# lenskit/csr

Measured on AMD Instinct MI355X. Metric: spmv_gflops, higher is better.
Workload: dtype f64

## Files before the change

### csr_amd/csrc/spmv.hip

```cpp
#include "spmv_plan.h"

#include <algorithm>
#include <ctime>

namespace csrk {
template <bool R32>
__device__ __forceinline__ double spmv_prod(double a, double x)
{
    const double t = a * x;
    return R32 ? (double)(float)t : t;
}

void free_spmv_plan(SpmvPlan *p) { delete p; }

void spmv_plan_bytes_by_part(const SpmvPlan *p, int64_t out[5])
{
    for (int i = 0; i < 5; i++) out[i] = 0;
    auto add = [&](int part, std::initializer_list<const DevBuf *> bufs) {
        for (const DevBuf *b : bufs) out[part] += (int64_t)b->bytes;
    };
    for (const AccPanel *ap : p->acc) add(0, {&ap->row_list, &ap->vals, &ap->idx, &ap->tile_row0, &ap->segs, &ap->wg_seg, &ap->partial, &ap->z});
    const Panel &t = p->tier1;
    add(1, {&t.row_list, &t.rp, &t.ci, &t.vs, &t.tile, &t.group, &t.carry_row, &t.carry_val, &t.y, &t.crp, &t.cidx});
    const LightStream *l = &p->ls;
// ... 369 lines not shown
                int q = atomicAdd(&s_nlong, 1);
                s_long[q] = r;
                continue;
            }
            double acc = ordered_sum(s_prod, s, e);
            if (r < nr) {
                yp[i0 + r] = acc;
            } else {
                *(pt.cslot >= 0 ? yp + pt.cslot : carry_val + t) = acc;
            }
        }
        __syncthreads();
        const int nlong = s_nlong;
        for (int q = wv; q < nlong; q += PT / WAVE) {
            int r = s_long[q];
            int s = r ? s_rend[r - 1] : 0;
            int e = s_rend[r];
            double acc = 0.0;
            for (int k = s + lane; k < e; k += WAVE) acc += s_prod[k];
            acc = wave_sum(acc);
            if (lane == 0) {
                if (r < nr) {
                    yp[i0 + r] = acc;
                } else {
                    *(pt.cslot >= 0 ? yp + pt.cslot : carry_val + t) = acc;
                }
            }
        }
        pt = nx;
    }
#undef PANEL_LOAD_TILE
}

typedef float f32x4_t __attribute__((ext_vector_type(4)));
template <class SV> struct AccVals;
template <> struct AccVals<double> {
    f64x2_t v[4];
    __device__ __forceinline__ void load(const double *tile, int lane)
    {
        const f64x2_t *vp = (const f64x2_t *)tile;
#pragma unroll
        for (int q = 0; q < 4; q++) v[q] = __builtin_nontemporal_load(vp + q * WAVE + lane);
    }
    __device__ __forceinline__ void get(double (&a)[ACC_K]) const
    {
#pragma unroll
        for (int q = 0; q < 4; q++) {
            a[2 * q] = v[q].x;
            a[2 * q + 1] = v[q].y;
        }
    }
};
template <> struct AccVals<float> {
    f32x4_t v[2];
    __device__ __forceinline__ void load(const float *tile, int lane)
    {
        const f32x4_t *vp = (const f32x4_t *)tile;
#pragma unroll
        for (int q = 0; q < 2; q++) v[q] = __builtin_nontemporal_load(vp + q * WAVE + lane);
    }
    __device__ __forceinline__ void get(double (&a)[ACC_K]) const
    {
#pragma unroll
        for (int q = 0; q < 2; q++) {
            a[4 * q] = (double)v[q].x;
            a[4 * q + 1] = (double)v[q].y;
            a[4 * q + 2] = (double)v[q].z;
            a[4 * q + 3] = (double)v[q].w;
        }
    }
};

template <int CB, int PT, bool R32 = false, class SV = double, class XT = double>
__global__ __launch_bounds__(PT) void spmv_acc_kernel(const SV *__restrict__ pvals, const uint16_t *__restrict__ pidx,
                                                     const int32_t *__restrict__ tile_row0,
                                                     const XT *__restrict__ x, int32_t ncols,
                                                     const AccSeg *__restrict__ segs, const int32_t *__restrict__ wg_seg,
                                                     int32_t H, double *__restrict__ partial)
{
    extern __shared__ __align__(16) unsigned char acc_smem[];
    double *s_x = (double *)acc_smem;
    double *s_acc = s_x + CB + 2;
    const int Hpad = (H + 1) & ~1;
    double *s_hval = s_acc + Hpad;
    int32_t *s_hrow = (int32_t *)(s_hval + ACC_SEG_TILES);
    constexpr int NW = PT / WAVE;
    const int tid = threadIdx.x, lane = tid & (WAVE - 1), wv = tid / WAVE;

    for (int h = tid; h < Hpad; h += PT) s_acc[h] = 0.0;
    if (tid < 2) s_x[CB + tid] = 0.0;
    const unsigned long long below = lane ? (~0ull >> (WAVE - lane)) : 0ull;
    const unsigned long long upto = below | (1ull << lane);

    int cur_blk = -1;
    const int sb = wg_seg[blockIdx.x], se = wg_seg[blockIdx.x + 1];
    for (int si = sb; si < se; si++) {
        const AccSeg sg = segs[si];
        if (sg.blk != cur_blk) {
            cur_blk = sg.blk;
            const int32_t w0 = sg.blk * CB;
            const int wlen = ncols - w0 < CB ? ncols - w0 : CB;
            if (wlen == CB) {
                constexpr int WL = CB / 2 / PT;
                f64x2_t v[WL];
#pragma unroll
                for (int u = 0; u < WL; u++) {
                    if (sizeof(XT) == 8) {
                        v[u] = *((const F64x2 *)(x + w0) + tid + u * PT);
                    } else {
                        const f32x2_t t = *((const F32x2 *)(x + w0) + tid + u * PT);
                        v[u].x = (double)t.x;
// ... 1 lines not shown
                    }
                }
#pragma unroll
                for (int u = 0; u < WL; u++) ((f64x2_t *)s_x)[tid + u * PT] = v[u];
            } else {
                for (int k = tid; k < wlen; k += PT) s_x[k] = (double)x[w0 + k];
            }
        }
        __syncthreads();

        const int nt = sg.ntiles;
        AccVals<SV> v, vn;
        u32x4_t ix, ixn;
        int32_t tr0 = 0, tr0n = 0;
        int t = wv;
        const int64_t pstep = (int64_t)gridDim.x;
        if (t < nt) {
            const u32x4_t *ip = (const u32x4_t *)(pidx + (sg.ptile0 + t * pstep) * ACC_TILE);
            v.load(pvals + (sg.ptile0 + t * pstep) * ACC_TILE, lane);
            ix = __builtin_nontemporal_load(ip + lane);
            tr0 = tile_row0[sg.tile0 + t];
        }
        for (; t < nt; t += NW) {
            const bool more = t + NW < nt;
            if (more) {
                const u32x4_t *ip = (const u32x4_t *)(pidx + (sg.ptile0 + (t + NW) * pstep) * ACC_TILE);
                vn.load(pvals + (sg.ptile0 + (t + NW) * pstep) * ACC_TILE, lane);
                ixn = __builtin_nontemporal_load(ip + lane);
                tr0n = tile_row0[sg.tile0 + t + NW];
            }
            const uint32_t e[ACC_K] = {ix.x & 0xffffu, ix.x >> 16, ix.y & 0xffffu, ix.y >> 16,
                                       ix.z & 0xffffu, ix.z >> 16, ix.w & 0xffffu, ix.w >> 16};
            double a[ACC_K];
            v.get(a);
            double xv[ACC_K];
#pragma unroll
            for (int j = 0; j < ACC_K; j++) xv[j] = s_x[e[j] & ACC_COL_MASK];
            int rw[ACC_K];
            {
                int lsum = 0;
#pragma unroll
                for (int j = 0; j < ACC_K; j++) lsum += (int)(e[j] >> ACC_ROW_SHIFT);
                int run = tr0 + wave_exscan_i32(lsum, lane);
#pragma unroll
                for (int j = 0; j < ACC_K; j++) {
                    run += (int)(e[j] >> ACC_ROW_SHIFT);
                    rw[j] = run;
                }
            }
            const int hr = rw[0];
            int cur = hr;
            double acc = 0.0, hs = 0.0;
            bool nb = false;
#pragma unroll
            for (int j = 0; j < ACC_K; j++) {
                const int r = rw[j];
                if (r != cur) {
                    if (!nb) {
                        hs = acc;
                        nb = true;
                    } else {
                        atomicAdd(&s_acc[cur], acc);
                    }
                    acc = 0.0;
                    cur = r;
                }
                if (R32) acc += spmv_prod<true>(a[j], xv[j]);
// ... 511 lines not shown
                dn[q] = k < k1 ? __builtin_nontemporal_load(a_dst + k) : 0;
            }
        }
#pragma unroll
        for (int q = 0; q < LS_STAGE_IPT; q++)
            if (c[q] >= 0) xg[d[q]] = s_x[c[q]];
        if (kn < k1) {
#pragma unroll
            for (int q = 0; q < LS_STAGE_IPT; q++) c[q] = cn[q], d[q] = dn[q];
        }
    }
}

int spmv_kernel_attributes()
{
    for (const void *f : {(const void *)spmv_acc_kernel<ACC_CB, ACC_THREADS>, (const void *)spmv_lstream_kernel<LS_PLAIN>,
                          (const void *)spmv_lstream_kernel<LS_RND>, (const void *)spmv_lstream_kernel<LS_PLAIN, true>,
                          (const void *)spmv_lstream_kernel<LS_RND, true>, (const void *)spmv_acc_kernel<ACC_CB, ACC_THREADS, true>,
                          (const void *)spmv_lstream_kernel<LS_PLAIN, false, true>, (const void *)spmv_lstream_kernel<LS_RND, false, true>,
                          (const void *)spmv_lstream_kernel<LS_PLAIN, true, true>, (const void *)spmv_lstream_kernel<LS_RND, true, true>,
                          (const void *)spmv_acc_kernel<ACC_CB, ACC_THREADS, false, float>,
                          (const void *)spmv_acc_kernel<ACC_CB, ACC_THREADS, true, float>,
                          (const void *)spmv_lstream_kernel<LS_PLAIN, false, false, float>, (const void *)spmv_lstream_kernel<LS_RND, false, false, float>,
                          (const void *)spmv_lstream_kernel<LS_PLAIN, true, false, float>, (const void *)spmv_lstream_kernel<LS_RND, true, false, float>,
                          (const void *)spmv_lstream_kernel<LS_PLAIN, false, true, float>, (const void *)spmv_lstream_kernel<LS_RND, false, true, float>,
                          (const void *)spmv_lstream_kernel<LS_PLAIN, true, true, float>, (const void *)spmv_lstream_kernel<LS_RND, true, true, float>,
                          (const void *)spmv_lstream_kernel<LS_RND24>, (const void *)spmv_lstream_kernel<LS_RND24, true>,
                          (const void *)spmv_lstream_kernel<LS_RND24, false, true>, (const void *)spmv_lstream_kernel<LS_RND24, true, true>,
                          (const void *)spmv_lstream_kernel<LS_RND24, false, false, float>, (const void *)spmv_lstream_kernel<LS_RND24, true, false, float>,
                          (const void *)spmv_lstream_kernel<LS_RND24, false, true, float>, (const void *)spmv_lstream_kernel<LS_RND24, true, true, float>,
                          (const void *)spmv_acc_kernel<ACC_CB, ACC_THREADS, false, double, float>,
                          (const void *)spmv_acc_kernel<ACC_CB, ACC_THREADS, true, double, float>,
                          (const void *)spmv_acc_kernel<ACC_CB, ACC_THREADS, false, float, float>,
                          (const void *)spmv_acc_kernel<ACC_CB, ACC_THREADS, true, float, float>})
        CSRK_HIP(hipFuncSetAttribute(f, hipFuncAttributeMaxDynamicSharedMemorySize, (int)(160 * 1024)));
    CSRK_HIP(hipFuncSetAttribute((const void *)ls_stage_kernel<double>, hipFuncAttributeMaxDynamicSharedMemorySize, (int)(LS_STAGE_WMAX * 8)));
    CSRK_HIP(hipFuncSetAttribute((const void *)ls_stage_kernel<float>, hipFuncAttributeMaxDynamicSharedMemorySize, (int)(LS_STAGE_WMAX * 8)));
    return CSRK_OK;
}

static int get_plan_locked(Matrix *m, hipStream_t s, SpmvPlan **out, bool launching)
{
    if (launching) m->spmv_calls++;
    const char *env = getenv("CSRK_SPMV_HEAVY_SPLIT"), *env_hot = getenv("CSRK_SPMV_HOT"), *env_ls = getenv("CSRK_SPMV_STREAM");
    const bool eager = (env && env[0] == '1') || (env_hot && env_hot[0] == '1') || (env_ls && env_ls[0] == '1') || !launching;
    const bool want_split = eager || m->spmv_calls >= 2;
    if (m->spmv_plan && !m->spmv_plan->split_considered && want_split && m->spmv_plan->algo == CSRK_SPMV_MERGE &&
        !m->spmv_plan->profiling) {
        if (hipDeviceSynchronize() != hipSuccess) {
            set_error("device synchronisation failed: %s", hipGetErrorString(hipGetLastError()));
            return CSRK_ERR_HIP;
        }
        free_spmv_plan(m->spmv_plan);
        m->spmv_plan = nullptr;
    }
    if (!m->spmv_plan) {
        SpmvPlan *p = new (std::nothrow) SpmvPlan();
        CSRK_REQUIRE(p, "out of host memory");
        p->algo = m->spmv_algo == CSRK_SPMV_AUTO ? CSRK_SPMV_MERGE : m->spmv_algo;
        (void)s;
        int rc = build_spmv_plan(m, p, want_split);
        if (rc == CSRK_OK && hipDeviceSynchronize() != hipSuccess) {
            set_error("SpMV plan construction failed: %s", hipGetErrorString(hipGetLastError()));
            rc = CSRK_ERR_HIP;
        }
        if (rc != CSRK_OK) {
            delete p;
// ... 54 lines not shown
            EpiJob J = {};
            J.kind = 1;
            J.blocks = (int32_t)ceil_div(H, WAVE * (EPI_THREADS / WAVE / G));
            J.partial = part;
            J.row_list = rows;
            J.H = H;
            J.n_wg = n_wg;
            J.G = G;
            J.extra = extra;
            J.crp = crp;
            J.cidx = cidx;
            J.cval = cval;
            epi.j[epi.n++] = J;
            return CSRK_OK;
        };
        if (do_light && p->ls.on && p->ls.n_cold) {
            KernelTimer ks(p, s, 3);
            const unsigned gs = (unsigned)(ceil_div(p->ls.n_stage_blk, 8) * 8);
            ls_stage_kernel<XT><<<gs, LS_STAGE_THREADS, (size_t)p->ls.stage_w * 8, s>>>(
                d_x, m->ncols, p->ls.stage_w, p->ls.a_col.as<uint16_t>(), p->ls.a_dst.as<int32_t>(),
                p->ls.blk_start.as<int32_t>(), p->ls.n_stage_blk, p->ls.xg.as<double>());
            ks.stop();
            CSRK_LAUNCH_CHECK();
        }
        if (do_light && p->n_hot && !(p->ls.on && p->ls.n_cold)) {
            hot_pack_kernel<XT><<<(unsigned)ceil_div(p->n_hot, 256), 256, 0, s>>>(d_x, p->hot_cols.as<int32_t>(), p->n_hot,
                                                                            p->xh.as<double>());
            CSRK_LAUNCH_CHECK();
        }
        bool t0_rides = false;
        if (do_heavy && p->n_heavy && !p->acc.empty()) {
            KernelTimer kh(p, s, 1);
            for (AccPanel *ap : p->acc) {
                if (ap->f32)
                    spmv_acc_kernel<ACC_CB, ACC_THREADS, R32, float, XT><<<(unsigned)ap->n_wg, ACC_THREADS, ap->lds, s>>>(
                        ap->vals.as<float>(), ap->idx.as<uint16_t>(), ap->tile_row0.as<int32_t>(), d_x, m->ncols,
                        ap->segs.as<AccSeg>(), ap->wg_seg.as<int32_t>(), ap->nrow, ap->partial.as<double>());
                else
                    spmv_acc_kernel<ACC_CB, ACC_THREADS, R32, double, XT><<<(unsigned)ap->n_wg, ACC_THREADS, ap->lds, s>>>(
                        ap->vals.as<double>(), ap->idx.as<uint16_t>(), ap->tile_row0.as<int32_t>(), d_x, m->ncols,
                        ap->segs.as<AccSeg>(), ap->wg_seg.as<int32_t>(), ap->nrow, ap->partial.as<double>());
                CSRK_LAUNCH_CHECK();
            }
            kh.stop();
        }
        if (do_heavy && p->n_heavy && p->tier1.on) {
            Panel *pn = &p->tier1;
            KernelTimer kh(p, s, 2);
#define PANEL_ARGS(PP)                                                                                              \
    pn->rp.as<PP>(), pn->ci.as<int32_t>(), pn->vs.as<double>(), d_x, m->ncols, pn->y.as<double>(),                    \
        pn->tile.as<PanelTile>(), pn->group.as<PanelGroup>(), pn->rows, pn->carry_row.as<int32_t>(),                  \
        pn->carry_val.as<double>(), pn->nnz, pn->cb, rider
            PanelRider rider = {pn->groups, nullptr, nullptr, 0, 0};
            if (PANEL_T1 / WAVE == 4 && do_heavy && p->acc.size() == 1 && p->acc[0]->z.p) {
                AccPanel *ap = p->acc[0];
                rider.partial = ap->partial.as<double>();
                rider.z = ap->z.as<double>();
                rider.H = ap->nrow;
                rider.n_wg = ap->n_wg;
                t0_rides = true;
            }
            const unsigned grid = (unsigned)(pn->groups + (t0_rides ? ceil_div(rider.H, WAVE) : 0));
            if (pn->p64) spmv_panel_kernel<int64_t, PANEL_T1, R32, XT><<<grid, PANEL_T1, 0, s>>>(PANEL_ARGS(int64_t));
            else spmv_panel_kernel<int32_t, PANEL_T1, R32, XT><<<grid, PANEL_T1, 0, s>>>(PANEL_ARGS(int32_t));
#undef PANEL_ARGS
            kh.stop();
            CSRK_LAUNCH_CHECK();
        }
        if (do_light) {
#define MERGE_ARGS_LIGHT(CI)                                                                                        \
    p->rp_light.as<P>(), CI, m->d_values, d_x, d_y, p->tile_row.as<int32_t>(), m->nrows, p->nnz_light,                \
        p->carry_row.as<int32_t>(), p->carry_val.as<double>(), p->tile_cut.as<int32_t>(), p->cut_pos.as<int64_t>(),  \
        p->cut_cum.as<int64_t>(), m->nnz
#define MERGE_ARGS_FULL(CI)                                                                                         \
// ... 457 lines not shown
```

### csr_amd/csrc/spmv_plan.h

```cpp
#pragma once
#include "common.h"
#include "wave.h"

#include <vector>

namespace csrk {

template <int VT> struct ValLoad;
template <> struct ValLoad<CSRK_VAL_F64> {
    static __device__ __forceinline__ double at(const void *v, int64_t k) { return ((const double *)v)[k]; }
};
template <> struct ValLoad<CSRK_VAL_F32> {
    static __device__ __forceinline__ double at(const void *v, int64_t k) { return (double)((const float *)v)[k]; }
};
template <> struct ValLoad<CSRK_VAL_NONE> {
    static __device__ __forceinline__ double at(const void *, int64_t) { return 1.0; }
};

__device__ __forceinline__ double wave_sum(double v)
{
#pragma unroll
    for (int off = WAVE / 2; off > 0; off >>= 1) v += __shfl_down(v, off, WAVE);
    return v;
}

__device__ __forceinline__ double ordered_sum(const double *p, int s, int e)
{
    double acc = 0.0;
    int k = s;
    for (; k + 4 <= e; k += 4) {
        const double a = p[k], b = p[k + 1], c = p[k + 2], d = p[k + 3];
        acc += a;
        acc += b;
        acc += c;
        acc += d;
    }
    for (; k < e; k++) acc += p[k];
    return acc;
}

struct Panel {
    bool on = false, p64 = false;
    int32_t cb = 0, nb = 0, nrow = 0;
    int64_t rows = 0, tiles = 0, nnz = 0, groups = 0;
    DevBuf row_list;
    DevBuf rp, ci, vs, tile, group, carry_row, carry_val, y;
    int32_t ncs = 0;
    DevBuf crp, cidx;
};

struct AccSeg {
    int64_t tile0;
    int64_t ptile0;
    int32_t ntiles;
    int32_t blk;
};

struct AccPanel {
    int32_t nrow = 0, nb = 0, n_wg = 0;
    int64_t tiles = 0, nnz = 0, n_segs = 0;
    size_t lds = 0;
    DevBuf row_list, vals, idx, tile_row0, segs, wg_seg, partial;
    DevBuf z;
    bool f32 = false;
};

struct LightStream {
    bool on = false;
    int64_t n_tiles = 0;
    int32_t n_runs = 0, n_out = 0;
    unsigned grid = 0;
    DevBuf vals, idx, rowids, tile_base, carry_row, carry_val;
    bool idx24 = false;
    bool f32 = false;
    bool dense = false;
    int64_t n_cold = 0;
    int32_t n_stage_blk = 0, stage_w = 0;
    DevBuf xg, a_col, a_dst, blk_start;
    int32_t stage_tiles = 0;
    DevBuf round_start, round_tile0, wg_round0;
};

struct SpmvPlan {
    int algo = CSRK_SPMV_MERGE;
    int tile_items = 0;
    int64_t n_tiles = 0;
    DevBuf tile_row;
    DevBuf carry_row;
    DevBuf carry_val;
    bool split_considered = false;
    int32_t n_heavy = 0;
    int32_t heavy_min = 0;
    int32_t tier1_min = 0;
    int64_t nnz_light = 0;
    DevBuf rp_light;
    DevBuf cut_pos;
    DevBuf cut_cum;
// ... 93 lines not shown
    int64_t t0;
    int32_t nt;
    int32_t blk;
};
constexpr int ACC_CB = 4096;
constexpr int ACC_K = 8;
constexpr int ACC_TILE = WAVE * ACC_K;
constexpr int ACC_MAXROWS = 15936;
constexpr int ACC_FLOOR = 128;
constexpr int ACC_SEG_TILES = 256;
constexpr int ACC_THREADS = 1024;
constexpr int ACC_ROW_SHIFT = 13;
constexpr uint32_t ACC_COL_MASK = (1u << ACC_ROW_SHIFT) - 1;
constexpr int ACC_MAXSTEP = 7;

typedef uint32_t u32x4_t __attribute__((ext_vector_type(4)));
typedef uint32_t u32x2_t __attribute__((ext_vector_type(2)));

__host__ __device__ __forceinline__ int acc_val_slot(int e)
{
    const int lane = e >> 3, j = e & 7;
    return (j >> 1) * (2 * WAVE) + lane * 2 + (j & 1);
}
__host__ __device__ __forceinline__ int acc_idx_slot(int e)
{
    const int lane = e >> 3, j = e & 7;
    return (j >> 2) * (4 * WAVE) + lane * 4 + (j & 3);
}
template <class SV> __host__ __device__ __forceinline__ int acc_slot_of(int e)
{
    return sizeof(SV) == 8 ? acc_val_slot(e) : acc_idx_slot(e);
}

#ifndef CSRK_LS_THREADS
#define CSRK_LS_THREADS 512
#endif
constexpr int LS_THREADS = CSRK_LS_THREADS;
#ifndef CSRK_LS_HOT_LDS
#define CSRK_LS_HOT_LDS 15360
#endif
constexpr int LS_HOT_LDS = CSRK_LS_HOT_LDS;
#ifndef CSRK_LS_RND_CAP
#define CSRK_LS_RND_CAP 8192
#endif
constexpr int LS_RND_CAP = CSRK_LS_RND_CAP, LS_RND_MAXTILES = 128;
constexpr int LS_RND_HOT = (160 * 1024 - (CSRK_LS_THREADS / 64) * (512 + 2) * 8) / 8 - LS_RND_CAP;
constexpr int LS_RID = 4;
#ifndef CSRK_LS_SEQ
#define CSRK_LS_SEQ 3
#endif
constexpr int LS_SEQ = CSRK_LS_SEQ;
constexpr uint32_t LS_HOT_BIT = 1u << 31, LS_START_BIT = 1u << 30, LS_COL_MASK = (1u << 30) - 1;
constexpr uint32_t LS_PAD = LS_COL_MASK;
#ifndef CSRK_LS_IDX24
#define CSRK_LS_IDX24 1
#endif
constexpr uint32_t LS24_HOT_BIT = 1u << 23, LS24_COL_MASK = (1u << 22) - 1;
constexpr int LS24_START_SHIFT = 22;
constexpr int64_t LS24_TILE_BYTES = 512 * 3;

constexpr int VEC_SEG = 4096;


#ifndef CSRK_STAGE_TILES
#define CSRK_STAGE_TILES 8
#endif
// ... 11 lines not shown
```

### csr_amd/csrc/spmv_plan.hip

```cpp
#include "spmv_plan.h"

#include <algorithm>
#include <cstring>
#include <ctime>

namespace csrk {
struct PlanTrace {
    bool on;
    double t0;
    static double now()
    {
        timespec ts;
        clock_gettime(CLOCK_MONOTONIC, &ts);
        return ts.tv_sec * 1e3 + ts.tv_nsec * 1e-6;
    }
    PlanTrace() : on(getenv("CSRK_PLAN_TRACE") != nullptr), t0(0.0)
    {
        if (on) {
            (void)hipDeviceSynchronize();
            t0 = now();
        }
    }
    void lap(const char *what)
    {
        if (!on) return;
        (void)hipDeviceSynchronize();
        const double t = now();
        fprintf(stderr, "[csrk plan] %-28s %8.3f ms\n", what, t - t0);
        t0 = t;
    }
};

template <class P>
__global__ void merge_plan_kernel(const P *__restrict__ rp, int32_t nrows, int64_t nnz, int items,
                                  int64_t n_tiles, int32_t *__restrict__ tile_row)
{
    int64_t t = (int64_t)blockIdx.x * blockDim.x + threadIdx.x;
// ... 461 lines not shown

__global__ __launch_bounds__(256) void acc_gap_kernel(int64_t *__restrict__ cnt, int32_t n_heavy, int32_t n_blocks,
                                                     int32_t *__restrict__ gap)
{
    const int64_t b = ((int64_t)blockIdx.x * blockDim.x + threadIdx.x) / WAVE;
    const int lane = threadIdx.x & (WAVE - 1);
    if (b >= n_blocks) return;
    int32_t last = -1;
    for (int32_t c0 = 0; c0 < n_heavy; c0 += WAVE) {
        const int32_t c = c0 + lane;
        const bool present = c < n_heavy && cnt[b * n_heavy + c] > 0;
        const unsigned long long mask = __ballot(present);
        const unsigned long long below = lane ? (mask & (~0ull >> (WAVE - lane))) : 0ull;
        const int32_t prev = below ? c0 + 63 - __clzll((long long)below) : last;
        if (c < n_heavy) {
            const int32_t g = present && prev >= 0 ? c - prev : 0;
            gap[b * n_heavy + c] = g;
            if (g > ACC_MAXSTEP) cnt[b * n_heavy + c] += (g - 1) / ACC_MAXSTEP;
        }
        if (mask) last = c0 + 63 - __clzll((long long)mask);
    }
}

__device__ __forceinline__ int64_t acc_phys_tile(int64_t t, const int64_t *__restrict__ wg_t0, int32_t n_wg)
{
    const int64_t n_tiles = wg_t0[n_wg];
    int64_t w = (int64_t)((double)t * (double)n_wg / (double)(n_tiles > 0 ? n_tiles : 1));
    w = w > n_wg - 1 ? n_wg - 1 : (w < 0 ? 0 : w);
    while (w > 0 && wg_t0[w] > t) w--;
    while (w + 1 < n_wg && wg_t0[w + 1] <= t) w++;
    return (t - wg_t0[w]) * n_wg + w;
}

template <class P, int VT, class SV>
__global__ __launch_bounds__(256) void acc_fill_kernel(const P *__restrict__ rp, const int32_t *__restrict__ ci,
                                                      const void *__restrict__ vs, const int32_t *__restrict__ heavy_row,
                                                      int32_t n_heavy, int32_t n_blocks, int32_t cb,
                                                      const int64_t *__restrict__ off, const int64_t *__restrict__ blk_tile0,
                                                      const int32_t *__restrict__ pstart, const int32_t *__restrict__ gap,
                                                      SV *__restrict__ pvals, uint16_t *__restrict__ pidx,
                                                      int32_t *__restrict__ tile_row0, const int64_t *__restrict__ wg_t0,
                                                      int32_t n_wg, int32_t waves_per_block)
{
    __shared__ int32_t s_start[256 / WAVE][WAVE];
    const int64_t w = ((int64_t)blockIdx.x * blockDim.x + threadIdx.x) / WAVE;
    const int lane = threadIdx.x & (WAVE - 1), wv = threadIdx.x / WAVE;
    const int32_t b = (int32_t)(w / waves_per_block);
    if (b >= n_blocks) return;
    const int32_t c0 = (int32_t)(w % waves_per_block) * WAVE, c = c0 + lane;
    const bool valid = c < n_heavy;
    const int64_t i = (int64_t)b * n_heavy + (valid ? c : c0);
    const int64_t off_i = off[i];
    int32_t n_all = 0, g = 0;
    int64_t lo = 0;
    if (valid) {
        n_all = (int32_t)(off[i + 1] - off_i);
        g = gap[i];
        lo = (int64_t)rp[heavy_row[c]] + pstart[i];
    }
    const int32_t npad = g > ACC_MAXSTEP ? (g - 1) / ACC_MAXSTEP : 0;
    const int32_t start = wave_exscan_i32(n_all, lane);
    const int32_t total = __builtin_amdgcn_readlane(start + n_all, WAVE - 1);
    if (total == 0) return;
    const int64_t L0 = blk_tile0[b] * ACC_TILE + (__shfl(off_i, 0, WAVE) - off[(int64_t)b * n_heavy]);
    int32_t *starts = s_start[wv];
    starts[lane] = start;
    __builtin_amdgcn_wave_barrier();
    for (int32_t d0 = 0; d0 < total; d0 += WAVE) {
        const int32_t d = d0 + lane;
        const bool in = d < total;
        int p = 0;
#pragma unroll
        for (int step = WAVE / 2; step; step >>= 1)
            if (in && starts[p + step] <= d) p += step;
        const int32_t at = d - __shfl(start, p, WAVE);
        const int32_t npad_p = __shfl(npad, p, WAVE), g_p = __shfl(g, p, WAVE);
        const int64_t lo_p = __shfl(lo, p, WAVE);
        if (!in) continue;
        const int64_t L = L0 + d;
        const int64_t t = L / ACC_TILE;
        const int el = (int)(L % ACC_TILE);
        const int64_t pt = acc_phys_tile(t, wg_t0, n_wg);
        if (at < npad_p) {
            pvals[pt * ACC_TILE + acc_slot_of<SV>(el)] = (SV)0.0;
            pidx[pt * ACC_TILE + el] = (uint16_t)((uint32_t)cb | ((el ? (uint32_t)ACC_MAXSTEP : 0u) << ACC_ROW_SHIFT));
            if (el == 0) tile_row0[t] = c0 + p - g_p + ACC_MAXSTEP * (at + 1);
        } else {
            const int64_t k = lo_p + (at - npad_p);
            const uint32_t step_in = at == npad_p ? (uint32_t)(g_p - ACC_MAXSTEP * npad_p) : 0u;
            pvals[pt * ACC_TILE + acc_slot_of<SV>(el)] = (SV)ValLoad<VT>::at(vs, k);
            pidx[pt * ACC_TILE + el] = (uint16_t)((uint32_t)(ci[k] - b * cb) | ((el ? step_in : 0u) << ACC_ROW_SHIFT));
            if (el == 0) tile_row0[t] = c0 + p;
        }
    }
}

template <class SV>
__global__ __launch_bounds__(256) void acc_pad_kernel(const int64_t *__restrict__ off, int32_t n_heavy, int32_t n_blocks,
                                                     const int64_t *__restrict__ blk_tile0, SV *__restrict__ pvals,
                                                     uint16_t *__restrict__ pidx, const int64_t *__restrict__ wg_t0, int32_t n_wg)
{
    const int32_t b = blockIdx.x;
    if (b >= n_blocks) return;
    const int64_t cnt = off[(int64_t)(b + 1) * n_heavy] - off[(int64_t)b * n_heavy];
    const int64_t L0 = blk_tile0[b] * ACC_TILE + cnt, L1 = blk_tile0[b + 1] * ACC_TILE;
    for (int64_t L = L0 + threadIdx.x; L < L1; L += blockDim.x) {
        const int64_t pt = acc_phys_tile(L / ACC_TILE, wg_t0, n_wg);
        const int el = (int)(L % ACC_TILE);
        pvals[pt * ACC_TILE + acc_slot_of<SV>(el)] = (SV)0.0;
        pidx[pt * ACC_TILE + el] = (uint16_t)ACC_CB;
    }
}


template <class P>
__device__ __forceinline__ int32_t ls_row_of(const P *__restrict__ rpv, int32_t nrows, int64_t L)
{
    int32_t lo = 0, hi = nrows - 1;
    while (lo < hi) {
        const int32_t mid = lo + ((hi - lo) >> 1);
        if ((int64_t)rpv[mid + 1] > L)
            hi = mid;
        else
            lo = mid + 1;
    }
    return lo;
}

template <class P>
__global__ void ls_tilerow_kernel(const P *__restrict__ rpv, int32_t nrows, int64_t n_ent, int64_t n_tiles, int32_t *__restrict__ tile_row)
{
    const int64_t t = (int64_t)blockIdx.x * blockDim.x + threadIdx.x;
    if (t > n_tiles) return;
    const int64_t e0 = t * ACC_TILE;
    tile_row[t] = t < n_tiles && e0 < n_ent ? ls_row_of(rpv, nrows, e0) : nrows - 1;
}

template <class P>
__global__ void ls_rowflag_kernel(const P *__restrict__ rpv, int32_t nrows, int32_t *__restrict__ flag)
{
    const int64_t r = (int64_t)blockIdx.x * blockDim.x + threadIdx.x;
    if (r <= nrows) flag[r] = (r < nrows && rpv[r + 1] > rpv[r]) ? 1 : 0;
}
// ... 252 lines not shown
    tr.lap("  tier 0: pair starts");
    acc_paircount_kernel<<<(unsigned)ceil_div(pairs, 256), 256, 0, s>>>(pstart.as<int32_t>(), pairs, n, off.as<int64_t>());
    CSRK_LAUNCH_CHECK();
    DevBuf gap;
    CSRK_TRY(gap.alloc((size_t)pairs * 4));
    acc_gap_kernel<<<(unsigned)ceil_div((int64_t)nb * WAVE, 256), 256, 0, s>>>(off.as<int64_t>(), n, nb, gap.as<int32_t>());
    CSRK_LAUNCH_CHECK();
    CSRK_TRY(exclusive_scan_i64(off.as<int64_t>(), off.as<int64_t>(), pairs, s));
    CSRK_TRY(bends.alloc((size_t)(nb + 1) * 8));
    panel_blockends_kernel<<<(unsigned)ceil_div(nb + 1, 256), 256, 0, s>>>(off.as<int64_t>(), n, nb, bends.as<int64_t>());
    CSRK_LAUNCH_CHECK();
    std::vector<int64_t> be((size_t)nb + 1), t0((size_t)nb + 1);
    CSRK_TRY(stage_d2h(be.data(), bends.p, (size_t)(nb + 1) * 8, s));
    CSRK_HIP(hipStreamSynchronize(s));
    t0[0] = 0;
    for (int32_t b = 0; b < nb; b++) t0[b + 1] = t0[b] + ceil_div(be[b + 1] - be[b], ACC_TILE);
    const int64_t n_tiles = t0[nb];
    CSRK_TRY(stage_h2d(bends.p, t0.data(), (size_t)(nb + 1) * 8, s));
    tr.lap("  tier 0: counts, gaps, scan");
    int cus = 0;
    CSRK_HIP(hipDeviceGetAttribute(&cus, hipDeviceAttributeMultiprocessorCount, m->device));
    int64_t n_wg = cus > 0 ? cus : 256;
    if (n_wg > n_tiles) n_wg = n_tiles;
    if (n_wg < 1) n_wg = 1;
    std::vector<int64_t> wg_t0((size_t)n_wg + 1);
    int64_t share_max = 0;
    for (int64_t w = 0; w <= n_wg; w++) wg_t0[(size_t)w] = n_tiles * w / n_wg;
    for (int64_t w = 0; w < n_wg; w++) share_max = std::max(share_max, wg_t0[(size_t)w + 1] - wg_t0[(size_t)w]);
    const int64_t n_phys = share_max * n_wg;
    DevBuf d_wg_t0;
    CSRK_TRY(d_wg_t0.alloc((size_t)(n_wg + 1) * 8));
    CSRK_TRY(stage_h2d(d_wg_t0.p, wg_t0.data(), (size_t)(n_wg + 1) * 8, s));
    ap->f32 = VT == CSRK_VAL_F32;
    CSRK_TRY(ap->vals.alloc((size_t)n_phys * ACC_TILE * (ap->f32 ? 4 : 8)));
    CSRK_TRY(ap->idx.alloc((size_t)n_phys * ACC_TILE * 2));
    CSRK_TRY(ap->tile_row0.alloc((size_t)(n_tiles ? n_tiles : 1) * 4));
    const int32_t fill_waves = (int32_t)ceil_div(n, WAVE);
#define ACC_FILL(SV)                                                                                                   \
    do {                                                                                                               \
        acc_fill_kernel<P, VT, SV><<<(unsigned)ceil_div((int64_t)nb * fill_waves * WAVE, 256), 256, 0, s>>>(           \
            rp, m->d_colinds, m->d_values, ap->row_list.as<int32_t>(), n, nb, ACC_CB, off.as<int64_t>(),               \
            bends.as<int64_t>(), pstart.as<int32_t>(), gap.as<int32_t>(), ap->vals.as<SV>(), ap->idx.as<uint16_t>(),   \
            ap->tile_row0.as<int32_t>(), d_wg_t0.as<int64_t>(), (int32_t)n_wg, fill_waves);                            \
        CSRK_LAUNCH_CHECK();                                                                                           \
        acc_pad_kernel<SV><<<(unsigned)nb, 256, 0, s>>>(off.as<int64_t>(), n, nb, bends.as<int64_t>(), ap->vals.as<SV>(), \
                                                        ap->idx.as<uint16_t>(), d_wg_t0.as<int64_t>(), (int32_t)n_wg); \
        CSRK_LAUNCH_CHECK();                                                                                           \
    } while (0)
    if (ap->f32) ACC_FILL(float);
    else ACC_FILL(double);
#undef ACC_FILL
    tr.lap("  tier 0: fill");
    std::vector<AccSeg> segs;
    std::vector<int32_t> wg_seg((size_t)n_wg + 1);
    int32_t b = 0;
    for (int64_t w = 0; w < n_wg; w++) {
        wg_seg[(size_t)w] = (int32_t)segs.size();
        int64_t t = wg_t0[(size_t)w];
        const int64_t t_end = wg_t0[(size_t)w + 1];
        while (t < t_end) {
            while (t0[b + 1] <= t) b++;
            int64_t e = t_end < t0[b + 1] ? t_end : t0[b + 1];
            if (e - t > ACC_SEG_TILES) e = t + ACC_SEG_TILES;
            AccSeg sg;
            sg.tile0 = t;
            sg.ptile0 = (t - wg_t0[(size_t)w]) * n_wg + w;
            sg.ntiles = (int32_t)(e - t);
            sg.blk = b;
            segs.push_back(sg);
            t = e;
        }
    }
    wg_seg[(size_t)n_wg] = (int32_t)segs.size();
    CSRK_TRY(ap->segs.alloc(segs.size() * sizeof(AccSeg)));
    CSRK_TRY(ap->wg_seg.alloc(wg_seg.size() * 4));
    CSRK_TRY(stage_h2d(ap->segs.p, segs.data(), segs.size() * sizeof(AccSeg), s));
    CSRK_TRY(stage_h2d(ap->wg_seg.p, wg_seg.data(), wg_seg.size() * 4, s));
    CSRK_TRY(ap->partial.alloc((size_t)n_wg * n * 8));
    CSRK_TRY(ap->z.alloc((size_t)n * 8));
    ap->lds = (size_t)(ACC_CB + 2) * 8 + (size_t)((n + 1) & ~1) * 8 + (size_t)ACC_SEG_TILES * 12;
    CSRK_TRY(spmv_kernel_attributes());
    CSRK_HIP(hipStreamSynchronize(s));
    ap->nrow = n;
    ap->nb = nb;
    ap->n_wg = (int32_t)n_wg;
// ... 788 lines not shown
```

Baseline: 775.7.

## Pack heavy-tier f64 values into lossless 56-bit fixed-point tiles

Adds a fix56 encoding for the heavy-row accumulator panel: at plan time a kernel scans the f64 values' exponent range, and if all values fit a shared 52-bit fixed-point grid they are stored as 7-byte split planes (lo/mid/hi) instead of 8-byte doubles. The SpMV kernel decodes them with a perm and magic-number subtraction. The goal is to cut value-stream bandwidth in this memory-bound kernel by 12.5%. A verify pass checks bit-exact roundtrip and falls back to plain doubles on mismatch, at the cost of extra plan time and some decode ALU work.

```diff
diff --git a/csr_amd/csrc/fix56.h b/csr_amd/csrc/fix56.h
--- /dev/null
+++ b/csr_amd/csrc/fix56.h
@@ -0,0 +1,119 @@
+#pragma once
+#include <cstdint>
+#include <cstring>
+
+#if defined(__HIPCC__)
+#define FIX56_HD __host__ __device__ __forceinline__
+#else
+#define FIX56_HD inline
+#endif
+
+namespace csrk {
+namespace fix56 {
+
+constexpr int TILE = 512;
+constexpr int LO_BYTES = TILE * 4, MID_BYTES = TILE * 2, HI_BYTES = TILE;
+constexpr int MID_OFF = LO_BYTES, HI_OFF = LO_BYTES + MID_BYTES;
+constexpr int TILE_BYTES = LO_BYTES + MID_BYTES + HI_BYTES;
+constexpr uint64_t MANT_MASK = (1ull << 52) - 1;
+constexpr uint32_t W_MANT = 0x000fffffu, W_SIGN = 0x00800000u;
+
+struct Packed {
+    unsigned char b[7];
+};
+static_assert(sizeof(Packed) * TILE == TILE_BYTES, "a tile of Packed entries is the three planes");
+
+FIX56_HD uint64_t bits_of(double v)
+{
+    uint64_t b;
+    memcpy(&b, &v, 8);
+    return b;
+}
+FIX56_HD double double_of(uint32_t hi, uint32_t lo)
+{
+    const uint64_t b = ((uint64_t)hi << 32) | lo;
+    double v;
+    memcpy(&v, &b, 8);
+    return v;
+}
+FIX56_HD int ctz64(uint64_t x) { return __builtin_ctzll(x); }
+FIX56_HD int msb64(uint64_t x) { return 63 - __builtin_clzll(x); }
+
+struct Range {
+    int32_t bad = 0, lo = INT32_MAX, hi = INT32_MIN;
+};
+FIX56_HD void split(uint64_t bits, uint64_t &sig, int &unit)
+{
+    const int e = (int)((bits >> 52) & 0x7ff);
+    sig = (bits & MANT_MASK) | (e ? 1ull << 52 : 0ull);
+    unit = (e ? e : 1) - 1075;
+}
+FIX56_HD void fold(Range &r, double v)
+{
+    const uint64_t b = bits_of(v);
+    if (b == 0) return;
+    if (((b >> 52) & 0x7ff) == 0x7ff || b == 1ull << 63) {
+        r.bad = 1;
+        return;
+    }
+    uint64_t sig;
+    int unit;
+    split(b, sig, unit);
+    const int lo = unit + ctz64(sig), hi = unit + msb64(sig);
+    r.lo = lo < r.lo ? lo : r.lo;
+    r.hi = hi > r.hi ? hi : r.hi;
+}
+FIX56_HD void merge(Range &r, const Range &o)
+{
+    r.bad |= o.bad;
+    r.lo = o.lo < r.lo ? o.lo : r.lo;
+    r.hi = o.hi > r.hi ? o.hi : r.hi;
+}
+FIX56_HD bool packable(const Range &r, int32_t &g)
+{
+    g = 0;
+    if (r.bad) return false;
+    if (r.lo > r.hi) return true;
+    g = r.lo;
+    return r.hi - g < 52 && 1075 + g >= 1 && 1075 + g <= 2046;
+}
+
+FIX56_HD uint64_t encode(double v, int32_t g)
+{
+    const uint64_t b = bits_of(v);
+    if ((b << 1) == 0) return 0;
+    uint64_t sig;
+    int unit;
+    split(b, sig, unit);
+    const uint64_t M = unit >= g ? sig << (unit - g) : sig >> (g - unit);
+    return M | (b >> 63) << 55;
+}
+FIX56_HD uint32_t lo_of(uint64_t p) { return (uint32_t)p; }
+FIX56_HD uint16_t mid_of(uint64_t p) { return (uint16_t)(p >> 32); }
+FIX56_HD unsigned char hi_of(uint64_t p) { return (unsigned char)(p >> 48); }
+
+FIX56_HD double decode(uint32_t lo, uint32_t w, uint32_t ebits, double magic)
+{
+    const double d = double_of((w & W_MANT) | ebits, lo) - magic;
+    return double_of((uint32_t)(bits_of(d) >> 32) ^ ((w & W_SIGN) << 8), (uint32_t)bits_of(d));
+}
+FIX56_HD uint32_t ebits_of(int32_t g) { return (uint32_t)(1075 + g) << 20; }
+FIX56_HD double magic_of(int32_t g) { return double_of(ebits_of(g), 0u); }
+
+FIX56_HD int lo_slot(int e) { return ((e & 7) >> 2) * 256 + (e >> 3) * 4 + (e & 3); }
+
+FIX56_HD void put(unsigned char *tile, int e, uint64_t p)
+{
+    ((uint32_t *)tile)[lo_slot(e)] = lo_of(p);
+    ((uint16_t *)(tile + MID_OFF))[e] = mid_of(p);
+    tile[HI_OFF + e] = hi_of(p);
+}
+FIX56_HD double get(const unsigned char *tile, int e, int32_t g)
+{
+    const uint32_t lo = ((const uint32_t *)tile)[lo_slot(e)];
+    const uint32_t w = (uint32_t)((const uint16_t *)(tile + MID_OFF))[e] | (uint32_t)tile[HI_OFF + e] << 16;
+    return decode(lo, w, ebits_of(g), magic_of(g));
+}
+
+}
+}
diff --git a/csr_amd/csrc/spmv.hip b/csr_amd/csrc/spmv.hip
--- a/csr_amd/csrc/spmv.hip
+++ b/csr_amd/csrc/spmv.hip
@@ -425,51 +425,12 @@
 #undef PANEL_LOAD_TILE
 }
 
-typedef float f32x4_t __attribute__((ext_vector_type(4)));
-template <class SV> struct AccVals;
-template <> struct AccVals<double> {
-    f64x2_t v[4];
-    __device__ __forceinline__ void load(const double *tile, int lane)
-    {
-        const f64x2_t *vp = (const f64x2_t *)tile;
-#pragma unroll
-        for (int q = 0; q < 4; q++) v[q] = __builtin_nontemporal_load(vp + q * WAVE + lane);
-    }
-    __device__ __forceinline__ void get(double (&a)[ACC_K]) const
-    {
-#pragma unroll
-        for (int q = 0; q < 4; q++) {
-            a[2 * q] = v[q].x;
-            a[2 * q + 1] = v[q].y;
-        }
-    }
-};
-template <> struct AccVals<float> {
-    f32x4_t v[2];
-    __device__ __forceinline__ void load(const float *tile, int lane)
-    {
-        const f32x4_t *vp = (const f32x4_t *)tile;
-#pragma unroll
-        for (int q = 0; q < 2; q++) v[q] = __builtin_nontemporal_load(vp + q * WAVE + lane);
-    }
-    __device__ __forceinline__ void get(double (&a)[ACC_K]) const
-    {
-#pragma unroll
-        for (int q = 0; q < 2; q++) {
-            a[4 * q] = (double)v[q].x;
-            a[4 * q + 1] = (double)v[q].y;
-            a[4 * q + 2] = (double)v[q].z;
-            a[4 * q + 3] = (double)v[q].w;
-        }
-    }
-};
-
 template <int CB, int PT, bool R32 = false, class SV = double, class XT = double>
 __global__ __launch_bounds__(PT) void spmv_acc_kernel(const SV *__restrict__ pvals, const uint16_t *__restrict__ pidx,
                                                      const int32_t *__restrict__ tile_row0,
                                                      const XT *__restrict__ x, int32_t ncols,
                                                      const AccSeg *__restrict__ segs, const int32_t *__restrict__ wg_seg,
-                                                     int32_t H, double *__restrict__ partial)
+                                                     int32_t H, double *__restrict__ partial, int32_t fx_g)
 {
     extern __shared__ __align__(16) unsigned char acc_smem[];
     double *s_x = (double *)acc_smem;
@@ -537,7 +498,7 @@
             const uint32_t e[ACC_K] = {ix.x & 0xffffu, ix.x >> 16, ix.y & 0xffffu, ix.y >> 16,
                                        ix.z & 0xffffu, ix.z >> 16, ix.w & 0xffffu, ix.w >> 16};
             double a[ACC_K];
-            v.get(a);
+            v.get(a, fx_g);
             double xv[ACC_K];
 #pragma unroll
             for (int j = 0; j < ACC_K; j++) xv[j] = s_x[e[j] & ACC_COL_MASK];
@@ -1115,7 +1076,11 @@
                           (const void *)spmv_acc_kernel<ACC_CB, ACC_THREADS, false, double, float>,
                           (const void *)spmv_acc_kernel<ACC_CB, ACC_THREADS, true, double, float>,
                           (const void *)spmv_acc_kernel<ACC_CB, ACC_THREADS, false, float, float>,
-                          (const void *)spmv_acc_kernel<ACC_CB, ACC_THREADS, true, float, float>})
+                          (const void *)spmv_acc_kernel<ACC_CB, ACC_THREADS, true, float, float>,
+                          (const void *)spmv_acc_kernel<ACC_CB, ACC_THREADS, false, fix56::Packed>,
+                          (const void *)spmv_acc_kernel<ACC_CB, ACC_THREADS, true, fix56::Packed>,
+                          (const void *)spmv_acc_kernel<ACC_CB, ACC_THREADS, false, fix56::Packed, float>,
+                          (const void *)spmv_acc_kernel<ACC_CB, ACC_THREADS, true, fix56::Packed, float>})
         CSRK_HIP(hipFuncSetAttribute(f, hipFuncAttributeMaxDynamicSharedMemorySize, (int)(160 * 1024)));
     CSRK_HIP(hipFuncSetAttribute((const void *)ls_stage_kernel<double>, hipFuncAttributeMaxDynamicSharedMemorySize, (int)(LS_STAGE_WMAX * 8)));
     CSRK_HIP(hipFuncSetAttribute((const void *)ls_stage_kernel<float>, hipFuncAttributeMaxDynamicSharedMemorySize, (int)(LS_STAGE_WMAX * 8)));
@@ -1236,14 +1201,14 @@
         if (do_heavy && p->n_heavy && !p->acc.empty()) {
             KernelTimer kh(p, s, 1);
             for (AccPanel *ap : p->acc) {
-                if (ap->f32)
-                    spmv_acc_kernel<ACC_CB, ACC_THREADS, R32, float, XT><<<(unsigned)ap->n_wg, ACC_THREADS, ap->lds, s>>>(
-                        ap->vals.as<float>(), ap->idx.as<uint16_t>(), ap->tile_row0.as<int32_t>(), d_x, m->ncols,
-                        ap->segs.as<AccSeg>(), ap->wg_seg.as<int32_t>(), ap->nrow, ap->partial.as<double>());
-                else
-                    spmv_acc_kernel<ACC_CB, ACC_THREADS, R32, double, XT><<<(unsigned)ap->n_wg, ACC_THREADS, ap->lds, s>>>(
-                        ap->vals.as<double>(), ap->idx.as<uint16_t>(), ap->tile_row0.as<int32_t>(), d_x, m->ncols,
-                        ap->segs.as<AccSeg>(), ap->wg_seg.as<int32_t>(), ap->nrow, ap->partial.as<double>());
+#define ACC_LAUNCH(SV)                                                                                                 \
+    spmv_acc_kernel<ACC_CB, ACC_THREADS, R32, SV, XT><<<(unsigned)ap->n_wg, ACC_THREADS, ap->lds, s>>>(                \
+        ap->vals.as<SV>(), ap->idx.as<uint16_t>(), ap->tile_row0.as<int32_t>(), d_x, m->ncols, ap->segs.as<AccSeg>(),  \
+        ap->wg_seg.as<int32_t>(), ap->nrow, ap->partial.as<double>(), ap->fx_g)
+                if (ap->f32) ACC_LAUNCH(float);
+                else if (ap->fix56) ACC_LAUNCH(fix56::Packed);
+                else ACC_LAUNCH(double);
+#undef ACC_LAUNCH
                 CSRK_LAUNCH_CHECK();
             }
             kh.stop();
diff --git a/csr_amd/csrc/spmv_plan.h b/csr_amd/csrc/spmv_plan.h
--- a/csr_amd/csrc/spmv_plan.h
+++ b/csr_amd/csrc/spmv_plan.h
@@ -1,6 +1,7 @@
 #pragma once
 #include "common.h"
 #include "wave.h"
+#include "fix56.h"
 
 #include <vector>
 
@@ -63,6 +64,8 @@
     DevBuf row_list, vals, idx, tile_row0, segs, wg_seg, partial;
     DevBuf z;
     bool f32 = false;
+    bool fix56 = false;
+    int32_t fx_g = 0;
 };
 
 struct LightStream {
@@ -222,6 +225,71 @@
     return sizeof(SV) == 8 ? acc_val_slot(e) : acc_idx_slot(e);
 }
 
+typedef float f32x4_t __attribute__((ext_vector_type(4)));
+template <class SV> struct AccVals;
+template <> struct AccVals<double> {
+    f64x2_t v[4];
+    __device__ __forceinline__ void load(const double *tile, int lane)
+    {
+        const f64x2_t *vp = (const f64x2_t *)tile;
+#pragma unroll
+        for (int q = 0; q < 4; q++) v[q] = __builtin_nontemporal_load(vp + q * WAVE + lane);
+    }
+    __device__ __forceinline__ void get(double (&a)[ACC_K], int32_t = 0) const
+    {
+#pragma unroll
+        for (int q = 0; q < 4; q++) {
+            a[2 * q] = v[q].x;
+            a[2 * q + 1] = v[q].y;
+        }
+    }
+};
+template <> struct AccVals<float> {
+    f32x4_t v[2];
+    __device__ __forceinline__ void load(const float *tile, int lane)
+    {
+        const f32x4_t *vp = (const f32x4_t *)tile;
+#pragma unroll
+        for (int q = 0; q < 2; q++) v[q] = __builtin_nontemporal_load(vp + q * WAVE + lane);
+    }
+    __device__ __forceinline__ void get(double (&a)[ACC_K], int32_t = 0) const
+    {
+#pragma unroll
+        for (int q = 0; q < 2; q++) {
+            a[4 * q] = (double)v[q].x;
+            a[4 * q + 1] = (double)v[q].y;
+            a[4 * q + 2] = (double)v[q].z;
+            a[4 * q + 3] = (double)v[q].w;
+        }
+    }
+};
+static_assert(fix56::TILE == ACC_TILE, "fix56 tiles are the streams' tiles");
+template <> struct AccVals<fix56::Packed> {
+    u32x4_t lo[2], mid;
+    u32x2_t hi;
+    __device__ __forceinline__ void load(const fix56::Packed *tile, int lane)
+    {
+        const unsigned char *tp = (const unsigned char *)tile;
+#pragma unroll
+        for (int q = 0; q < 2; q++) lo[q] = __builtin_nontemporal_load((const u32x4_t *)tp + q * WAVE + lane);
+        mid = __builtin_nontemporal_load((const u32x4_t *)(tp + fix56::MID_OFF) + lane);
+        hi = __builtin_nontemporal_load((const u32x2_t *)(tp + fix56::HI_OFF) + lane);
+    }
+    __device__ __forceinline__ void get(double (&a)[ACC_K], int32_t g) const
+    {
+        const uint32_t l[ACC_K] = {lo[0].x, lo[0].y, lo[0].z, lo[0].w, lo[1].x, lo[1].y, lo[1].z, lo[1].w};
+        const uint32_t m[4] = {mid.x, mid.y, mid.z, mid.w}, h[2] = {hi.x, hi.y};
+        const uint32_t ebits = fix56::ebits_of(g);
+        const double magic = fix56::magic_of(g);
+#pragma unroll
+        for (int j = 0; j < ACC_K; j++) {
+            const uint32_t w = __builtin_amdgcn_perm(h[j >> 2], m[j >> 1],
+                                                     0x0c000000u | ((4u + (j & 3)) << 16) | ((2u * (j & 1) + 1u) << 8) | (2u * (j & 1)));
+            a[j] = fix56::decode(l[j], w, ebits, magic);
+        }
+    }
+};
+
 #ifndef CSRK_LS_THREADS
 #define CSRK_LS_THREADS 512
 #endif
diff --git a/csr_amd/csrc/spmv_plan.hip b/csr_amd/csrc/spmv_plan.hip
--- a/csr_amd/csrc/spmv_plan.hip
+++ b/csr_amd/csrc/spmv_plan.hip
@@ -3,6 +3,7 @@
 #include <algorithm>
 #include <cstring>
 #include <ctime>
+#include <type_traits>
 
 namespace csrk {
 struct PlanTrace {
@@ -530,7 +531,51 @@
     return (t - wg_t0[w]) * n_wg + w;
 }
 
-template <class P, int VT, class SV>
+template <class P>
+__global__ __launch_bounds__(256) void acc_range_kernel(const P *__restrict__ rp, const double *__restrict__ vs,
+                                                       const int32_t *__restrict__ rows, int32_t *__restrict__ out)
+{
+    const int32_t row = rows[blockIdx.x];
+    const int64_t k1 = (int64_t)rp[row + 1];
+    fix56::Range r;
+    for (int64_t k = (int64_t)rp[row] + blockIdx.y * 256 + threadIdx.x; k < k1; k += (int64_t)gridDim.y * 256) fix56::fold(r, vs[k]);
+#pragma unroll
+    for (int off = WAVE / 2; off > 0; off >>= 1) {
+        fix56::Range o;
+        o.bad = __shfl_xor(r.bad, off, WAVE);
+        o.lo = __shfl_xor(r.lo, off, WAVE);
+        o.hi = __shfl_xor(r.hi, off, WAVE);
+        fix56::merge(r, o);
+    }
+    if ((threadIdx.x & (WAVE - 1)) == 0) {
+        const volatile int32_t *seen = out;
+        if (r.bad && !seen[0]) atomicOr(out, 1);
+        if (r.lo < seen[1]) atomicMin(out + 1, r.lo);
+        if (r.hi > seen[2]) atomicMax(out + 2, r.hi);
+    }
+}
+
+template <class SV, bool VERIFY>
+__device__ __forceinline__ void acc_put(SV *__restrict__ pvals, int64_t pt, int el, double v, int32_t fx_g,
+                                        int32_t *__restrict__ mismatch)
+{
+    if constexpr (!std::is_same<SV, fix56::Packed>::value) {
+        pvals[pt * ACC_TILE + acc_slot_of<SV>(el)] = (SV)v;
+    } else if constexpr (!VERIFY) {
+        fix56::put((unsigned char *)(pvals + pt * ACC_TILE), el, fix56::encode(v, fx_g));
+    } else {
+        AccVals<SV> t;
+        t.load(pvals + pt * ACC_TILE, el >> 3);
+        double a[ACC_K];
+        t.get(a, fx_g);
+        double d = a[0];
+#pragma unroll
+        for (int j = 1; j < ACC_K; j++) d = (el & 7) == j ? a[j] : d;
+        if (fix56::bits_of(d) != fix56::bits_of(v)) *mismatch = 1;
+    }
+}
+
+template <class P, int VT, class SV, bool VERIFY = false>
 __global__ __launch_bounds__(256) void acc_fill_kernel(const P *__restrict__ rp, const int32_t *__restrict__ ci,
                                                       const void *__restrict__ vs, const int32_t *__restrict__ heavy_row,
                                                       int32_t n_heavy, int32_t n_blocks, int32_t cb,
@@ -538,7 +583,8 @@
                                                       const int32_t *__restrict__ pstart, const int32_t *__restrict__ gap,
                                                       SV *__restrict__ pvals, uint16_t *__restrict__ pidx,
                                                       int32_t *__restrict__ tile_row0, const int64_t *__restrict__ wg_t0,
-                                                      int32_t n_wg, int32_t waves_per_block)
+                                                      int32_t n_wg, int32_t waves_per_block, int32_t fx_g,
+                                                      int32_t *__restrict__ mismatch)
 {
     __shared__ int32_t s_start[256 / WAVE][WAVE];
     const int64_t w = ((int64_t)blockIdx.x * blockDim.x + threadIdx.x) / WAVE;
@@ -580,23 +626,26 @@
         const int el = (int)(L % ACC_TILE);
         const int64_t pt = acc_phys_tile(t, wg_t0, n_wg);
         if (at < npad_p) {
-            pvals[pt * ACC_TILE + acc_slot_of<SV>(el)] = (SV)0.0;
+            acc_put<SV, VERIFY>(pvals, pt, el, 0.0, fx_g, mismatch);
+            if (VERIFY) continue;
             pidx[pt * ACC_TILE + el] = (uint16_t)((uint32_t)cb | ((el ? (uint32_t)ACC_MAXSTEP : 0u) << ACC_ROW_SHIFT));
             if (el == 0) tile_row0[t] = c0 + p - g_p + ACC_MAXSTEP * (at + 1);
         } else {
             const int64_t k = lo_p + (at - npad_p);
             const uint32_t step_in = at == npad_p ? (uint32_t)(g_p - ACC_MAXSTEP * npad_p) : 0u;
-            pvals[pt * ACC_TILE + acc_slot_of<SV>(el)] = (SV)ValLoad<VT>::at(vs, k);
+            acc_put<SV, VERIFY>(pvals, pt, el, ValLoad<VT>::at(vs, k), fx_g, mismatch);
+            if (VERIFY) continue;
             pidx[pt * ACC_TILE + el] = (uint16_t)((uint32_t)(ci[k] - b * cb) | ((el ? step_in : 0u) << ACC_ROW_SHIFT));
             if (el == 0) tile_row0[t] = c0 + p;
         }
     }
 }
 
-template <class SV>
+template <class SV, bool VERIFY = false>
 __global__ __launch_bounds__(256) void acc_pad_kernel(const int64_t *__restrict__ off, int32_t n_heavy, int32_t n_blocks,
                                                      const int64_t *__restrict__ blk_tile0, SV *__restrict__ pvals,
-                                                     uint16_t *__restrict__ pidx, const int64_t *__restrict__ wg_t0, int32_t n_wg)
+                                                     uint16_t *__restrict__ pidx, const int64_t *__restrict__ wg_t0, int32_t n_wg,
+                                                     int32_t fx_g, int32_t *__restrict__ mismatch)
 {
     const int32_t b = blockIdx.x;
     if (b >= n_blocks) return;
@@ -605,8 +654,8 @@
     for (int64_t L = L0 + threadIdx.x; L < L1; L += blockDim.x) {
         const int64_t pt = acc_phys_tile(L / ACC_TILE, wg_t0, n_wg);
         const int el = (int)(L % ACC_TILE);
-        pvals[pt * ACC_TILE + acc_slot_of<SV>(el)] = (SV)0.0;
-        pidx[pt * ACC_TILE + el] = (uint16_t)ACC_CB;
+        acc_put<SV, VERIFY>(pvals, pt, el, 0.0, fx_g, mismatch);
+        if (!VERIFY) pidx[pt * ACC_TILE + el] = (uint16_t)ACC_CB;
     }
 }
 
@@ -925,25 +974,64 @@
     CSRK_TRY(d_wg_t0.alloc((size_t)(n_wg + 1) * 8));
     CSRK_TRY(stage_h2d(d_wg_t0.p, wg_t0.data(), (size_t)(n_wg + 1) * 8, s));
     ap->f32 = VT == CSRK_VAL_F32;
-    CSRK_TRY(ap->vals.alloc((size_t)n_phys * ACC_TILE * (ap->f32 ? 4 : 8)));
+    DevBuf fx;
+    CSRK_TRY(fx.alloc(16));
+    if (VT == CSRK_VAL_F64 && n > 0) {
+        const char *env = getenv("CSRK_SPMV_FIX56");
+        if (!(env && env[0] == '0')) {
+            int32_t h[4] = {0, INT32_MAX, INT32_MIN, 0};
+            CSRK_TRY(stage_h2d(fx.p, h, sizeof h, s));
+            acc_range_kernel<P><<<dim3((unsigned)n, 16), 256, 0, s>>>(rp, (const double *)m->d_values, ap->row_list.as<int32_t>(),
+                                                                     fx.as<int32_t>());
+            CSRK_LAUNCH_CHECK();
+            CSRK_TRY(stage_d2h(h, fx.p, sizeof h, s));
+            CSRK_HIP(hipStreamSynchronize(s));
+            fix56::Range r;
+            r.bad = h[0];
+            r.lo = h[1];
+            r.hi = h[2];
+            ap->fix56 = fix56::packable(r, ap->fx_g);
+            tr.lap("  tier 0: value grid test");
+        }
+    }
     CSRK_TRY(ap->idx.alloc((size_t)n_phys * ACC_TILE * 2));
     CSRK_TRY(ap->tile_row0.alloc((size_t)(n_tiles ? n_tiles : 1) * 4));
     const int32_t fill_waves = (int32_t)ceil_div(n, WAVE);
-#define ACC_FILL(SV)                                                                                                   \
+#define ACC_FILL(SV, VERIFY)                                                                                           \
     do {                                                                                                               \
-        acc_fill_kernel<P, VT, SV><<<(unsigned)ceil_div((int64_t)nb * fill_waves * WAVE, 256), 256, 0, s>>>(           \
+        acc_fill_kernel<P, VT, SV, VERIFY><<<(unsigned)ceil_div((int64_t)nb * fill_waves * WAVE, 256), 256, 0, s>>>(   \
             rp, m->d_colinds, m->d_values, ap->row_list.as<int32_t>(), n, nb, ACC_CB, off.as<int64_t>(),               \
             bends.as<int64_t>(), pstart.as<int32_t>(), gap.as<int32_t>(), ap->vals.as<SV>(), ap->idx.as<uint16_t>(),   \
-            ap->tile_row0.as<int32_t>(), d_wg_t0.as<int64_t>(), (int32_t)n_wg, fill_waves);                            \
+            ap->tile_row0.as<int32_t>(), d_wg_t0.as<int64_t>(), (int32_t)n_wg, fill_waves, ap->fx_g,                   \
+            fx.as<int32_t>() + 3);                                                                                     \
         CSRK_LAUNCH_CHECK();                                                                                           \
-        acc_pad_kernel<SV><<<(unsigned)nb, 256, 0, s>>>(off.as<int64_t>(), n, nb, bends.as<int64_t>(), ap->vals.as<SV>(), \
-                                                        ap->idx.as<uint16_t>(), d_wg_t0.as<int64_t>(), (int32_t)n_wg); \
+        acc_pad_kernel<SV, VERIFY><<<(unsigned)nb, 256, 0, s>>>(off.as<int64_t>(), n, nb, bends.as<int64_t>(),         \
+                                                                ap->vals.as<SV>(), ap->idx.as<uint16_t>(),             \
+                                                                d_wg_t0.as<int64_t>(), (int32_t)n_wg, ap->fx_g,        \
+                                                                fx.as<int32_t>() + 3);                                 \
         CSRK_LAUNCH_CHECK();                                                                                           \
     } while (0)
-    if (ap->f32) ACC_FILL(float);
-    else ACC_FILL(double);
+    if (ap->fix56) {
+        CSRK_TRY(ap->vals.alloc((size_t)n_phys * fix56::TILE_BYTES));
+        ACC_FILL(fix56::Packed, false);
+        tr.lap("  tier 0: fill (fix56)");
+        int32_t mismatch = 1;
+        ACC_FILL(fix56::Packed, true);
+        CSRK_TRY(stage_d2h(&mismatch, fx.as<int32_t>() + 3, 4, s));
+        CSRK_HIP(hipStreamSynchronize(s));
+        tr.lap("  tier 0: verify (fix56)");
+        if (mismatch) {
+            ap->fix56 = false;
+            ap->fx_g = 0;
+        }
+    }
+    if (!ap->fix56) {
+        CSRK_TRY(ap->vals.alloc((size_t)n_phys * ACC_TILE * (ap->f32 ? 4 : 8)));
+        if (ap->f32) ACC_FILL(float, false);
+        else ACC_FILL(double, false);
+        tr.lap("  tier 0: fill");
+    }
 #undef ACC_FILL
-    tr.lap("  tier 0: fill");
     std::vector<AccSeg> segs;
     std::vector<int32_t> wg_seg((size_t)n_wg + 1);
     int32_t b = 0;
```

Result: faster. 798.3, median of 6 (+2.9%).
